# privacy-scaling-explorations/snark-verifier

Hardware: AMD Instinct MI355X
Metric: BN254 G1 MSM points/sec at 2^20 (higher is better)
Workload: dtype i32x9 (254-bit Montgomery Fq as 9 x 29-bit limbs on the integer VALU); 1 GPU; BN254 G1 Pippenger MSM, 2^20 random points/scalars per GPU, inputs resident in HBM, affine result (configs[1]); points_per_gpu=1048576, points_per_kernel_launch=1048576, window_bits=default, msms_in_flight=264

## Files before the change

### snark-verifier_amd/csrc/ctx.hpp

```cpp
#pragma once
#include <hip/hip_runtime.h>
#include <mutex>
#include <stddef.h>
#include <stdint.h>
#include <stdio.h>
#include "../../include/snarkv_amd.h"
#include "curve_consts.h"

#if defined(SNARKV_CURVE_PALLAS)
#define SNARKV_API(name) snarkv_pallas_##name
#define SNARKV_CHUNK_PIPELINE 0
#define SNARKV_API_FLAGS SNARKV_FLAG_VALIDATE
#else
#define SNARKV_API(name) snarkv_##name
#define SNARKV_CHUNK_PIPELINE 1
#define SNARKV_API_FLAGS (SNARKV_FLAG_VALIDATE | SNARKV_FLAG_MONTGOMERY)
#endif

namespace snarkv {

void set_last_error(const char* fmt, ...);

#define SNARKV_HIP(expr)                                                                   \
  do {                                                                                     \
// ... 32 lines not shown
  SLOT_MISC,
  SLOT_SORT_TMP,
  SLOT_SHIFTED,
  SLOT_GLV,
  SLOT_FIX_LISTS,
  SLOT_MISC2,
  SLOT_TERM_CHAIN,
  SLOT_TERM_MAGS,
  SLOT_SPLIT_PARTIALS,
  SLOT_IPA_XI,
  SLOT_IPA_H,
  SLOT_IPA_OUT,
  SLOT_MGPU_GRID,
  SLOT_MGPU_RECV,
  SLOT_IPA_FOLD,
  SLOT_POLY,
  SLOT_NTT,
  SLOT_POLY_PROD,
  SLOT_COUNT
};

}

struct snarkv_ctx {
  int device;
  hipStream_t stream;
  bool own_stream;
  void* buf[snarkv::SLOT_COUNT];
  size_t cap[snarkv::SLOT_COUNT];
  void* hbuf[SNARKV_HOST_BUFFERS];
  size_t hbuf_cap[SNARKV_HOST_BUFFERS];
  uint32_t flags;
  bool mont;
  bool stage_timing;
  float stage_ms[SNARKV_PIP_STAGES];
  hipEvent_t ev[SNARKV_PIP_STAGES + 1];
  bool ev_ready;
  snarkv_ctx* sub[4];
  hipEvent_t sub_ev[5];
  bool sub_ready;
  hipEvent_t sorted_ev;
  bool sorted_ev_ready;
  int last_split_workers;
  bool throughput_mode;
  int throughput_peers;
  bool is_lane;
  snarkv_ctx* jobs[SNARKV_MANY_MAX_JOBS];
  int njobs;
  int last_many_jobs;
  size_t many_sig;
  hipStream_t copy_stream;
  bool copy_ready;
  hipEvent_t many_ev[2];
  hipEvent_t order_ev;
  bool order_ev_ready;
  hipStream_t hi_stream[2];
  bool hi_ready;
  void* ntt_tables;
  uint32_t ntt_key;
};

struct snarkv_dk {
  int device;
// ... 32 lines not shown
  explicit WireFormScope(snarkv_ctx* ctx) : c(ctx), saved(ctx ? ctx->mont : false) {
    if (c) c->mont = false;
  }
  ~WireFormScope() {
    if (c) c->mont = saved;
  }
};
#define SNARKV_WIRE_FORM(ctx) ::snarkv::WireFormScope _wire_form((ctx))

int ctx_reserve(snarkv_ctx* ctx, int slot, size_t bytes, void** out);
int stage_in(snarkv_ctx* ctx, int slot, const void* host, size_t bytes, void** d);
int fetch_out(snarkv_ctx* ctx, const void* d, void* host, size_t bytes);
int check_validate(snarkv_ctx* ctx, const void* d_s, const void* d_p, size_t n, uint32_t flags);
int ctx_lanes(snarkv_ctx* ctx);
int ctx_lanes_fork(snarkv_ctx* ctx);
int ctx_lanes_join(snarkv_ctx* ctx);
inline snarkv_ctx* ctx_lane(snarkv_ctx* ctx, size_t i) { return (i % 4 == 3) ? ctx : ctx->sub[i % 4]; }

int launch_msm_batched(snarkv_ctx* ctx, const void* d_scalars, const void* d_points, const void* d_offsets,
                       size_t n_msm, size_t n_terms, void* d_out);
int launch_g1_decompress(snarkv_ctx* ctx, const void* d_in32, size_t n, void* d_out64, void* d_ok);
int launch_msm_pippenger(snarkv_ctx* ctx, const void* d_scalars, const void* d_points, size_t n, int window_bits,
                         void* d_out, bool partial_out, void* d_buckets_out = nullptr);
enum { PIP_PHASE_SORT = 1, PIP_PHASE_ACC = 2, PIP_PHASE_TAIL = 4, PIP_PHASE_ALL = 7 };
int launch_msm_pippenger_phases(snarkv_ctx* ctx, hipStream_t st, int phases, const void* d_scalars, const void* d_points,
                                size_t n, int window_bits, void* d_out, bool partial_out, void* d_buckets_out,
                                void* d_grid);
int launch_buckets_reduce_many(snarkv_ctx* ctx, hipStream_t st, const void* d_grids, uint32_t c, uint32_t windows,
                               uint32_t jobs, void* d_out, bool partial_out);
int launch_msm_pippenger_many(snarkv_ctx* ctx, size_t count, const void* const* d_scalars, const void* const* d_points,
                              const size_t* n, int window_bits, void* d_out, bool partial_out, hipEvent_t* ready = nullptr);
int launch_msm_pippenger_auto(snarkv_ctx* ctx, const void* d_scalars, const void* d_points, size_t n, int window_bits,
                              void* d_out, bool partial_out);
bool pip_chunk_pipeline(size_t n, int window_bits, bool is_lane, size_t* chunk);
int msm_pippenger_staged(snarkv_ctx* ctx, const uint8_t* scalars32, const uint8_t* points64, size_t n, uint32_t flags,
                         uint8_t out64[64]);
int pip_geometry(size_t n_total, int window_bits, uint32_t* c, uint32_t* windows, uint32_t* buckets_per_window);
int launch_buckets_add(snarkv_ctx* ctx, void* d_dst, const void* d_src, size_t count);
int launch_buckets_reduce(snarkv_ctx* ctx, const void* d_buckets, uint32_t c, uint32_t w0, uint32_t wcount, void* d_partial);
int launch_fold_partials(snarkv_ctx* ctx, const void* d_partials, size_t count, void* d_out64, bool partial_out = false);
int launch_fold_partials_many(snarkv_ctx* ctx, const void* d_partials, size_t count, size_t jobs, void* d_out64s);
constexpr size_t kSharedTableCap = (size_t)256 << 20;
bool ipa_dk_table_fits(const snarkv_ipa_dk* dk);
int ipa_dk_table_prepare(snarkv_ctx* ctx, const snarkv_ipa_dk* dk, bool* have);
int launch_msm_shared(snarkv_ctx* ctx, const snarkv_ipa_dk* dk, const void* d_scalars, size_t n, size_t m, uint32_t slices,
                      void* d_out64s);
int launch_validate(snarkv_ctx* ctx, const void* d_scalars, const void* d_points, size_t n, int* bad_host);
int launch_g2_prepare(snarkv_ctx* ctx, const void* d_g2x2_256, void* d_prep);
int launch_decide(snarkv_ctx* ctx, const void* d_prep, const void* d_accs, size_t m, void* d_ok, void* d_gt);
int launch_validate_g2(snarkv_ctx* ctx, const void* d_g2x2_256, int* bad_host);
// ... 7 lines not shown
```

### snark-verifier_amd/csrc/msm_api.hip

```cpp
#include <stdlib.h>
#include <algorithm>
#include "ctx.hpp"
#include "../../include/snarkv_pallas.h"

namespace snarkv {

bool pip_chunk_pipeline(size_t n, int window_bits, bool is_lane, size_t* chunk) {
  const size_t c = (size_t)1 << 20;
  const char* e = getenv("SNARKV_PIP_SPLIT");
  const int mode = e ? atoi(e) : 1;
  const size_t min_chunks = mode == 2 ? 2 : 3;
  if (chunk) *chunk = c;
  return SNARKV_CHUNK_PIPELINE && mode != 0 && (n + c - 1) / c >= min_chunks && window_bits == 0 && !is_lane;
}

int launch_msm_pippenger_auto(snarkv_ctx* ctx, const void* d_s, const void* d_p, size_t n, int window_bits, void* d_out,
                              bool partial_out) {
  size_t kChunk = 0;
  const bool split = pip_chunk_pipeline(n, window_bits, ctx->is_lane, &kChunk);
  const size_t chunks = (n + kChunk - 1) / kChunk;
  ctx->last_split_workers = 0;
  ctx->last_many_jobs = 0;
  if (!split) return launch_msm_pippenger(ctx, d_s, d_p, n, window_bits, d_out, partial_out);
  SNARKV_TRY(ctx_lanes(ctx));
  const bool tm = ctx->stage_timing;
  if (tm && !ctx->ev_ready) {
// ... 96 lines not shown
    for (int i = 0; i <= SNARKV_PIP_STAGES; ++i) SNARKV_HIP(hipEventCreate(&ctx->ev[i]));
    ctx->ev_ready = true;
  }
  if (sig != ctx->many_sig) {
    SNARKV_HIP(hipDeviceSynchronize());
    ctx->many_sig = sig;
  }
  hipStream_t S[3] = {ctx->stream, ctx->sub[0]->stream, ctx->sub[1]->stream};
  constexpr int nS = 3;
  auto join_and_fork = [&]() -> int {
    for (int k = 0; k < 2; ++k) {
      SNARKV_HIP(hipEventRecord(ctx->many_ev[k], ctx->hi_stream[k]));
      SNARKV_HIP(hipStreamWaitEvent(ctx->stream, ctx->many_ev[k], 0));
    }
    for (int k = 0; k + 1 < nS; ++k) {
      SNARKV_HIP(hipEventRecord(ctx->sub_ev[k], S[k + 1]));
      SNARKV_HIP(hipStreamWaitEvent(ctx->stream, ctx->sub_ev[k], 0));
    }
    SNARKV_HIP(hipEventRecord(ctx->sub_ev[4], ctx->stream));
    for (int k = 0; k < 2; ++k) SNARKV_HIP(hipStreamWaitEvent(ctx->hi_stream[k], ctx->sub_ev[4], 0));
    for (int k = 0; k + 1 < nS; ++k) SNARKV_HIP(hipStreamWaitEvent(S[k + 1], ctx->sub_ev[4], 0));
    return SNARKV_OK;
  };
  void* d_grids = nullptr;
  const size_t grid_bytes = (size_t)w0 * b0 * SNARKV_G1_PARTIAL_BYTES;
  if (uniform) SNARKV_TRY(ctx_reserve(ctx, SLOT_MGPU_GRID, grid_bytes * G, &d_grids));
  if (tm) SNARKV_HIP(hipEventRecord(ctx->ev[0], ctx->stream));
  SNARKV_TRY(join_and_fork());
  for (size_t lo = 0; lo < count; lo += G) {
    const size_t hi = std::min(count, lo + G);
    const bool last = hi == count;
    for (size_t i = lo; i < hi; ++i) {
      snarkv_ctx* job = ctx->jobs[i - lo];
      job->mont = ctx->mont;
      job->stage_timing = tm && last;
      void* grid = uniform ? (uint8_t*)d_grids + grid_bytes * (i - lo) : nullptr;
      hipStream_t sa = ctx->hi_stream[(i - lo) % 2], sb = S[(i - lo) % nS];
      if (ready) SNARKV_HIP(hipStreamWaitEvent(sa, ready[i], 0));
      SNARKV_TRY(launch_msm_pippenger_phases(job, sa, PIP_PHASE_SORT, d_s[i], d_p[i], n[i], window_bits, nullptr, false,
                                             nullptr, grid));
      SNARKV_HIP(hipEventRecord(job->sorted_ev, sa));
      SNARKV_HIP(hipStreamWaitEvent(sb, job->sorted_ev, 0));
      SNARKV_TRY(launch_msm_pippenger_phases(job, sb, PIP_PHASE_ACC, d_s[i], d_p[i], n[i], window_bits, nullptr, false,
                                             nullptr, grid));
      if (!uniform)
        SNARKV_TRY(launch_msm_pippenger_phases(job, sb, PIP_PHASE_TAIL, d_s[i], d_p[i], n[i], window_bits,
                                               (uint8_t*)d_out + ostride * i, partial_out, nullptr, nullptr));
      job->stage_timing = false;
    }
    SNARKV_TRY(join_and_fork());
    if (uniform) {
      SNARKV_TRY(launch_buckets_reduce_many(ctx, ctx->stream, d_grids, c0, w0, (uint32_t)(hi - lo),
                                            (uint8_t*)d_out + ostride * lo, partial_out));
      if (!last) SNARKV_TRY(join_and_fork());
    }
    if (last) ctx->last_many_jobs = (int)(hi - lo);
  }
  if (tm) SNARKV_HIP(hipEventRecord(ctx->ev[SNARKV_PIP_STAGES - 1], ctx->stream));
  return SNARKV_OK;
}

int msm_pippenger_staged(snarkv_ctx* ctx, const uint8_t* scalars32, const uint8_t* points64, size_t n, uint32_t flags,
                         uint8_t out64[64]) {
  if (!ctx || !scalars32 || !points64 || !out64) return SNARKV_ERR_ARG;
  if (n == 0) return SNARKV_ERR_EMPTY;
  SNARKV_HIP(hipSetDevice(ctx->device));
  SNARKV_CALL_FLAGS(ctx, flags & SNARKV_API_FLAGS);
  void *d_s, *d_p, *d_out;
  SNARKV_TRY(stage_in(ctx, SLOT_IN_SCALARS, scalars32, n * 32, &d_s));
  SNARKV_TRY(stage_in(ctx, SLOT_IN_POINTS, points64, n * 64, &d_p));
  SNARKV_TRY(ctx_reserve(ctx, SLOT_OUT, 64, &d_out));
  SNARKV_TRY(check_validate(ctx, d_s, d_p, n, flags));
  SNARKV_TRY(launch_msm_pippenger_auto(ctx, d_s, d_p, n, 0, d_out, false));
// ... 49 lines not shown
```

### snark-verifier_amd/csrc/msm_pippenger.hip

```cpp
#include <stdlib.h>
#include <string.h>
#include <algorithm>
#include <mutex>
#include <atomic>
#include "ctx.hpp"
#include "g1_29.h"
#include "fr29.h"
#ifndef SNARKV_GLV
#define SNARKV_GLV 1
#endif
#if SNARKV_GLV
#include "glv.h"
#endif

namespace snarkv {

#ifndef SNARKV_KRUN
#define SNARKV_KRUN 128
#endif
#ifndef SNARKV_KCHUNK
#define SNARKV_KCHUNK 8
#endif
#ifndef SNARKV_TILE_THREADS
#define SNARKV_TILE_THREADS 256
// ... 116 lines not shown
    k[4 * j + 1] = q.y;
    k[4 * j + 2] = q.z;
    k[4 * j + 3] = q.w;
  }
#if SNARKV_GLV
  uint32_t sgn = k[3] >> 31;
  k[3] &= 0x7FFFFFFFu;
  return sgn;
#else
  return 0u;
#endif
}

__device__ __forceinline__ uint32_t xcd_tile(uint32_t b, uint32_t nblk) {
#if SNARKV_XCD_TILES
  return (nblk & 7u) == 0 ? (b & 7u) * (nblk >> 3) + (b >> 3) : b;
#else
  return b;
#endif
}

__global__ void __launch_bounds__(SNARKV_PREP_THREADS)
    k_prepare(const uint32_t* __restrict__ scalars, const uint32_t* __restrict__ points,
              G1Packed* __restrict__ pts, uint4* __restrict__ glv, PipParams p, uint32_t* __restrict__ M) {
  SNARKV_RAISE_PRIO();
  extern __shared__ uint32_t lds[];
  for (uint32_t k = threadIdx.x; k < p.nkeys; k += blockDim.x) lds[k] = 0u;
  __syncthreads();
  const uint32_t tile = xcd_tile(blockIdx.x, p.nblk);
  uint32_t lo = tile * p.tile;
  uint32_t hi = lo + p.tile < p.n ? lo + p.tile : p.n;
  for (uint32_t i = lo + threadIdx.x; i < hi; i += blockDim.x) {
    const uint4* s = reinterpret_cast<const uint4*>(points + (size_t)i * 16);
    uint32_t w[16];
#pragma unroll
    for (int j = 0; j < 4; ++j) {
      uint4 v = s[j];
      w[4 * j] = v.x;
      w[4 * j + 1] = v.y;
      w[4 * j + 2] = v.z;
      w[4 * j + 3] = v.w;
    }
    G1Affine29 a = g1a29_from_words(w, p.mont != 0);
    bool ident = g1a29_is_identity(a);
    pts[kHalves * (size_t)i] = g1a29_pack(a);
    const uint4* ks = reinterpret_cast<const uint4*>(scalars + (size_t)i * 8);
    uint4 k0 = ks[0], k1 = ks[1];
// ... 13 lines not shown
    pts[2 * (size_t)i + 1] = g1a29_pack(a);
    glv_decompose(k, o);
#else
#pragma unroll
    for (int j = 0; j < 8; ++j) o[j] = k[j];
#endif
    if (ident) {
#pragma unroll
      for (int j = 0; j < 8; ++j) o[j] = 0;
    }
    glv[2 * (size_t)i] = make_uint4(o[0], o[1], o[2], o[3]);
    glv[2 * (size_t)i + 1] = make_uint4(o[4], o[5], o[6], o[7]);
#pragma unroll
    for (int h = 0; h < kHalves; ++h) {
      uint32_t d[kDigitWords];
      uint32_t sgn = load_digit_words(o + h * kDigitWords, d);
      for_each_digit(d, sgn, p, [&](uint32_t key, uint32_t, uint32_t) { atomicAdd(&lds[key], 1u); });
    }
  }
  __syncthreads();
  for (uint32_t k = threadIdx.x; k < p.nkeys; k += blockDim.x) M[(size_t)k * p.mstride + tile] = lds[k];
  if (blockIdx.x == 0 && p.mstride > p.nblk)
    for (uint32_t k = threadIdx.x; k < p.nkeys; k += blockDim.x) M[(size_t)k * p.mstride + p.nblk] = 0u;
}

constexpr uint32_t kStageScalars = SNARKV_TILE_BASE;
constexpr uint32_t kStageItems = kStageScalars / SNARKV_TILE_THREADS;
static_assert(kStageScalars % SNARKV_TILE_THREADS == 0, "a staged tile gives every lane the same number of scalars");
__global__ void __launch_bounds__(SNARKV_TILE_THREADS) SNARKV_SCATTER_ATTR
    k_sort_scatter_staged(const uint4* __restrict__ glv, PipParams p, const uint32_t* __restrict__ M,
                          uint2* __restrict__ tmp) {
  SNARKV_RAISE_PRIO();
  extern __shared__ uint32_t lds[];
  uint32_t* gbase = lds;
  uint32_t* cnt = lds + p.SB;
  uint32_t* off = lds + 2 * p.SB;
  uint32_t* wsum = lds + 3 * p.SB;
  uint2* stage = reinterpret_cast<uint2*>(lds + 3 * p.SB + 16 + (p.SB & 1u));
  const uint32_t tid = threadIdx.x, lane = tid & 63u, wave = tid >> 6;
  const uint32_t tile = xcd_tile(blockIdx.x, p.nblk);
  const uint32_t lo = tile * kStageScalars;
  const uint32_t hi = lo + kStageScalars < p.n ? lo + kStageScalars : p.n;
  const uint32_t per = (p.SB + SNARKV_TILE_THREADS - 1) / SNARKV_TILE_THREADS;
  for (int w = 0; w < p.W; ++w) {
    for (uint32_t k = tid; k < p.SB; k += blockDim.x) {
      gbase[k] = M[((size_t)w * p.SB + k) * p.mstride + tile];
// ... 182 lines not shown
    for (int j = 0; j < kPer; ++j) {
      uint32_t e = threadIdx.x + j * T;
      if (e < cnt_items) stage[atomicAdd(&hist[mine[j].x & low_mask], 1u)] = mine[j];
    }
    __syncthreads();
    for (uint32_t e = threadIdx.x; e < cnt_items; e += T) entries[begin + e] = stage[e];
  } else {
    for (uint32_t e = begin + threadIdx.x; e < end; e += T) {
      uint2 it = tmp[e];
      entries[begin + atomicAdd(&hist[it.x & low_mask], 1u)] = it;
    }
  }
}

constexpr uint32_t kSchedBuckets = 2048;
constexpr uint32_t kMaxPiece = 256;
constexpr uint32_t kBigPieces = 24;
constexpr uint32_t kFixGrid = 1024;
constexpr uint32_t kPieceWhole = 0x80000000u;
__host__ __device__ constexpr uint32_t sched_rows(uint32_t L) { return L + 3; }

__global__ void __launch_bounds__(256)
    k_piece_hist(const uint32_t* __restrict__ counts, PipParams p, uint32_t nsb, uint32_t* __restrict__ H,
                 uint32_t* __restrict__ misc) {
  SNARKV_RAISE_PRIO();
  __shared__ uint32_t hist[sched_rows(kMaxPiece)];
  const uint32_t L = p.krun, rows = sched_rows(L);
  for (uint32_t k = threadIdx.x; k < rows; k += blockDim.x) hist[k] = 0u;
  if (blockIdx.x == 0 && threadIdx.x == 0) misc[4] = 0u;
  __syncthreads();
  const uint32_t lo = blockIdx.x * kSchedBuckets, hi = lo + kSchedBuckets < p.nb ? lo + kSchedBuckets : p.nb;
  for (uint32_t b = lo + threadIdx.x; b < hi; b += blockDim.x) {
    const uint32_t c = counts[b];
    if (c <= L) {
      atomicAdd(&hist[L - c], 1u);
      continue;
    }
    const uint32_t nfull = c / L, r = c - nfull * L;
    atomicAdd(&hist[0], nfull);
    if (r) atomicAdd(&hist[L - r], 1u);
    atomicAdd(&hist[nfull + (r ? 1u : 0u) > kBigPieces ? L + 2 : L + 1], 1u);
  }
  __syncthreads();
  for (uint32_t k = threadIdx.x; k < rows; k += blockDim.x) H[(size_t)k * nsb + blockIdx.x] = hist[k];
}

__global__ void __launch_bounds__(256)
    k_piece_emit(const uint32_t* __restrict__ counts, const uint32_t* __restrict__ offsets, PipParams p, uint32_t nsb,
                 const uint32_t* __restrict__ H, uint32_t split_slots, uint4* __restrict__ pieces,
                 uint32_t* __restrict__ small_list, uint32_t* __restrict__ big_list) {
  SNARKV_RAISE_PRIO();
  __shared__ uint32_t cur[sched_rows(kMaxPiece)];
  const uint32_t L = p.krun, rows = sched_rows(L);
  for (uint32_t k = threadIdx.x; k < rows; k += blockDim.x) cur[k] = H[(size_t)k * nsb + blockIdx.x];
  const uint32_t small0 = H[(size_t)(L + 1) * nsb], big0 = H[(size_t)(L + 2) * nsb];
  __syncthreads();
  const uint32_t lo = blockIdx.x * kSchedBuckets, hi = lo + kSchedBuckets < p.nb ? lo + kSchedBuckets : p.nb;
  for (uint32_t b = lo + threadIdx.x; b < hi; b += blockDim.x) {
    const uint32_t c = counts[b], o = offsets[b];
    if (c <= L) {
      pieces[atomicAdd(&cur[L - c], 1u)] = make_uint4(o, c | kPieceWhole, b, 0u);
      continue;
    }
    const uint32_t nfull = c / L, r = c - nfull * L, slot = o / L;
    const uint32_t at = atomicAdd(&cur[0], nfull);
    for (uint32_t j = 0; j < nfull; ++j) pieces[at + j] = make_uint4(o + j * L, L, b, slot + j);
    if (r) pieces[atomicAdd(&cur[L - r], 1u)] = make_uint4(o + nfull * L, r, b, split_slots + slot);
    if (nfull + (r ? 1u : 0u) > kBigPieces) big_list[atomicAdd(&cur[L + 2], 1u) - big0] = b;
    else small_list[atomicAdd(&cur[L + 1], 1u) - small0] = b;
  }
}

constexpr uint32_t kEntryIdx = 0x7FFFFFFFu;

__device__ __forceinline__ G1Affine29 entry_point(const G1Packed& k, uint32_t y) {
  G1Affine29 p = g1a29_unpack(k);
  if (y >> 31) p.y = fq29_neg(p.y);
  return p;
}
// ... 56 lines not shown
    const uint32_t i = atomicAdd(deg_count, 1u);
    if (i < p.nb) deg_list[i] = b;
  } else {
    buckets[b] = acc;
  }
}

__device__ __noinline__ void bucket_from_entries_careful(const uint2* __restrict__ entries, const G1Packed* __restrict__ pts,
                                                         uint32_t o, uint32_t cnt, uint32_t first, uint32_t stride,
                                                         bool sanitize, G1Xyzz29* out) {
  G1Xyzz29 acc = xyzz29_identity();
  for (uint32_t e = o + first; e < o + cnt; e += stride) {
    uint2 ent = entries[e];
    G1Affine29 p = entry_point(pts[ent.y & kEntryIdx], ent.y);
    xyzz29_madd_careful(acc, p);
  }
  *out = sanitize ? xyzz29_sanitize(acc) : acc;
}

__device__ __forceinline__ uint32_t piece_slot(uint32_t o, uint32_t j, uint32_t nfull, uint32_t L, uint32_t split_slots) {
  return j < nfull ? o / L + j : split_slots + o / L;
}

__global__ void __launch_bounds__(256)
    k_fixup(const uint32_t* __restrict__ counts, const uint32_t* __restrict__ offsets, const uint2* __restrict__ entries,
            const G1Packed* __restrict__ pts, const G1Xyzz29* __restrict__ parts, uint32_t split_slots,
            G1Xyzz29* __restrict__ buckets, const uint32_t* __restrict__ H, uint32_t nsb, const uint32_t* __restrict__ misc,
            const uint32_t* __restrict__ small_list, const uint32_t* __restrict__ big_list,
            const uint32_t* __restrict__ deg_list, PipParams p) {
  SNARKV_RAISE_PRIO();
  __shared__ G1Xyzz29 sh[256];
  __shared__ int any_bad;
  const uint32_t L = p.krun;
  const uint32_t small0 = H[(size_t)(L + 1) * nsb], big0 = H[(size_t)(L + 2) * nsb];
  const uint32_t nsmall = big0 - small0, nbig = misc[6] - big0;
  const uint32_t ndeg = misc[4] < p.nb ? misc[4] : p.nb;
  for (uint32_t bi = blockIdx.x; bi < nbig; bi += gridDim.x) {
    const uint32_t b = big_list[bi];
    const uint32_t o = offsets[b], cnt = counts[b], nfull = cnt / L, np = nfull + (cnt % L ? 1u : 0u);
    if (threadIdx.x == 0) any_bad = 0;
    __syncthreads();
    G1Xyzz29 acc = xyzz29_identity();
    bool bad = false;
    for (uint32_t j = threadIdx.x; j < np; j += blockDim.x) {
      const G1Xyzz29 part = parts[piece_slot(o, j, nfull, L, split_slots)];
      bad = bad || xyzz29_is_degenerate(part);
      xyzz29_add_careful(acc, part);
    }
    if (bad) atomicOr(&any_bad, 1);
    __syncthreads();
    if (any_bad) bucket_from_entries_careful(entries, pts, o, cnt, threadIdx.x, blockDim.x, false, &sh[threadIdx.x]);
    else sh[threadIdx.x] = acc;
    __syncthreads();
    for (uint32_t st = 128; st >= 1; st >>= 1) {
      if (threadIdx.x < st) {
        G1Xyzz29 a = sh[threadIdx.x];
        xyzz29_add_careful(a, sh[threadIdx.x + st]);
        sh[threadIdx.x] = a;
      }
      __syncthreads();
    }
    if (threadIdx.x == 0) buckets[b] = xyzz29_sanitize(sh[0]);
    __syncthreads();
  }
  for (uint32_t i = blockIdx.x * blockDim.x + threadIdx.x; i < nsmall + ndeg; i += gridDim.x * blockDim.x) {
    const bool split = i < nsmall;
    const uint32_t b = split ? small_list[i] : deg_list[i - nsmall];
    const uint32_t o = offsets[b], cnt = counts[b];
    bool bad = !split;
    G1Xyzz29 acc = xyzz29_identity();
    if (split) {
      const uint32_t nfull = cnt / L, np = nfull + (cnt % L ? 1u : 0u);
      for (uint32_t j = 0; j < np; ++j) {
        const G1Xyzz29 part = parts[piece_slot(o, j, nfull, L, split_slots)];
        bad = bad || xyzz29_is_identity(part);
        xyzz29_add_skipid_fast(acc, part, bad);
      }
      bad = bad || xyzz29_is_degenerate(acc);
    }
    if (bad) bucket_from_entries_careful(entries, pts, o, cnt, 0, 1, true, &buckets[b]);
    else buckets[b] = acc;
  }
}

__device__ __forceinline__ G1Xyzz29 xyzz29_sel(bool c, const G1Xyzz29& a, const G1Xyzz29& b) {
  G1Xyzz29 r;
#pragma unroll
  for (int i = 0; i < 9; ++i) {
    r.x.v[i] = c ? a.x.v[i] : b.x.v[i];
    r.y.v[i] = c ? a.y.v[i] : b.y.v[i];
    r.zz.v[i] = c ? a.zz.v[i] : b.zz.v[i];
    r.zzz.v[i] = c ? a.zzz.v[i] : b.zzz.v[i];
  }
  return r;
}

template <bool CAREFUL>
__device__ __forceinline__ bool chunk_sums(const G1Xyzz29* __restrict__ bw, uint32_t base, uint32_t top,
                                           G1Xyzz29& run, G1Xyzz29& acc) {
  run = xyzz29_identity();
  acc = xyzz29_identity();
  bool bad = false;
#pragma unroll 1
  for (uint32_t op = 0; op < 2 * (top - base); ++op) {
    bool second = op & 1u;
// ... 209 lines not shown
  while (high < p.c - 1 && ((kHalves * n) >> (high + 1)) >= kSortTarget && ((uint64_t)p.W << (high + 1)) <= kMaxKeys) ++high;
  p.low_bits = (p.c - 1) - high;
  p.SB = p.B >> p.low_bits;
  p.nkeys = (uint32_t)p.W * p.SB;
  p.tile = SNARKV_TILE_BASE;
  static_assert(kStageItems * kHalves <= 32, "a staged lane keeps one sign bit per entry in a 32-bit word");
  const size_t lds_staged = ((size_t)3 * p.SB + 16 + (p.SB & 1u)) * 4 + (size_t)kStageScalars * kHalves * 8;
  p.nblk = (uint32_t)((n + p.tile - 1) / p.tile);
  p.mstride = p.nblk | 1u;
  uint64_t max_entries = (uint64_t)kHalves * (uint64_t)n * (uint64_t)p.W;
  if (n == 0 || max_entries >= 0xFFFFFFFFull || n >= 0x40000000ull) {
    set_last_error("pippenger: n=%zu out of range", n);
    return SNARKV_ERR_LENGTH;
  }
  if ((size_t)p.nkeys * 4 > 65536 || lds_staged > 96 * 1024) {
    set_last_error("pippenger: key table too large (nkeys=%u)", p.nkeys);
    return SNARKV_ERR_LENGTH;
  }
  p.krun = ctx->throughput_mode ? (uint32_t)kRunThroughput : latency_run_length(max_entries);
  const uint32_t max_pieces = (uint32_t)std::min<uint64_t>((uint64_t)p.nb + max_entries / p.krun, 0xFFFFFFFFull - 63);
  const uint32_t split_slots = (uint32_t)(max_entries / p.krun) + 1;
  const uint32_t nsb = (p.nb + kSchedBuckets - 1) / kSchedBuckets;
  const uint32_t hcount = sched_rows(p.krun) * nsb;
  const uint32_t hscan_blocks = (hcount + 1023) / 1024;
  uint32_t mcount = p.nkeys * p.mstride;
  uint32_t scan_blocks = (mcount + 1023) / 1024;
  uint32_t chunks_per_window = (p.B + kChunk - 1) / kChunk;
  uint32_t blocks_per_window = (chunks_per_window + 63) / 64;

  void *d_pts, *d_glv, *d_counts, *d_offsets, *d_M, *d_blocksum, *d_entries, *d_tmp, *d_pieces, *d_hist, *d_parts,
      *d_buckets, *d_wave, *d_shift, *d_misc, *d_lists;
  SNARKV_TRY(ctx_reserve(ctx, SLOT_POINTS_MONT, kHalves * n * sizeof(G1Packed), &d_pts));
  SNARKV_TRY(ctx_reserve(ctx, SLOT_GLV, n * 32, &d_glv));
  SNARKV_TRY(ctx_reserve(ctx, SLOT_COUNTS, (size_t)p.nb * 4, &d_counts));
  SNARKV_TRY(ctx_reserve(ctx, SLOT_OFFSETS, (size_t)p.nb * 4, &d_offsets));
  SNARKV_TRY(ctx_reserve(ctx, SLOT_CURSOR, (size_t)mcount * 4, &d_M));
  SNARKV_TRY(ctx_reserve(ctx, SLOT_BLOCKSUMS, (size_t)std::max(scan_blocks, hscan_blocks) * 4 + 64, &d_blocksum));
  SNARKV_TRY(ctx_reserve(ctx, SLOT_ENTRIES, max_entries * 8, &d_entries));
  SNARKV_TRY(ctx_reserve(ctx, SLOT_SORT_TMP, max_entries * 8, &d_tmp));
  SNARKV_TRY(ctx_reserve(ctx, SLOT_PIECES, (size_t)max_pieces * sizeof(uint4), &d_pieces));
  SNARKV_TRY(ctx_reserve(ctx, SLOT_PIECE_HIST, (size_t)hcount * 4, &d_hist));
  SNARKV_TRY(ctx_reserve(ctx, SLOT_SPLIT_PARTS, (size_t)split_slots * 2 * sizeof(G1Xyzz29), &d_parts));
  if (d_grid) d_buckets = d_grid;
  else SNARKV_TRY(ctx_reserve(ctx, SLOT_BUCKETS, (size_t)p.nb * sizeof(G1Xyzz29), &d_buckets));
  SNARKV_TRY(ctx_reserve(ctx, SLOT_CHUNK_PARTIALS, 2 * (size_t)blocks_per_window * p.W * sizeof(G1Xyzz29), &d_wave));
  SNARKV_TRY(ctx_reserve(ctx, SLOT_SHIFTED, (size_t)p.W * sizeof(G1Xyzz29), &d_shift));
  SNARKV_TRY(ctx_reserve(ctx, SLOT_MISC, 64, &d_misc));
  SNARKV_TRY(ctx_reserve(ctx, SLOT_FIX_LISTS, (size_t)p.nb * 3 * 4, &d_lists));
  uint32_t* d_total = (uint32_t*)d_misc;
  uint32_t* d_small = (uint32_t*)d_lists, *d_bigl = d_small + p.nb, *d_deg = d_bigl + p.nb;
  const uint32_t* d_npieces = (const uint32_t*)d_hist + (size_t)(p.krun + 1) * nsb;

  const bool tm = ctx->stage_timing && phases == PIP_PHASE_ALL;
  const bool tm_acc = ctx->stage_timing && phases == PIP_PHASE_ACC;
  int evi = 0;
#define STAGE_MARK()                                         \
  do {                                                       \
    if (tm) SNARKV_HIP(hipEventRecord(ctx->ev[evi++], st));  \
  } while (0)
  if ((tm || tm_acc) && !ctx->ev_ready) {
    for (int i = 0; i <= SNARKV_PIP_STAGES; ++i) SNARKV_HIP(hipEventCreate(&ctx->ev[i]));
    ctx->ev_ready = true;
  }
  STAGE_MARK();
  if (phases & PIP_PHASE_SORT) {
    hipLaunchKernelGGL(k_prepare, dim3(p.nblk), dim3(SNARKV_PREP_THREADS), (size_t)p.nkeys * 4, st, (const uint32_t*)d_scalars,
                       (const uint32_t*)d_points, (G1Packed*)d_pts, (uint4*)d_glv, p, (uint32_t*)d_M);
    STAGE_MARK();
    hipLaunchKernelGGL(k_scan_local, dim3(scan_blocks), dim3(256), 0, st, (uint32_t*)d_M, (uint32_t*)d_blocksum, mcount);
    hipLaunchKernelGGL(k_scan_blocksums, dim3(1), dim3(1024), 0, st, (uint32_t*)d_blocksum, scan_blocks, d_total);
    hipLaunchKernelGGL(k_scan_add, dim3(scan_blocks), dim3(256), 0, st, (uint32_t*)d_M, (const uint32_t*)d_blocksum,
                       mcount);
    STAGE_MARK();
    static std::atomic<uint64_t> attr_set{0};
    const uint64_t bit = 1ull << (ctx->device & 63);
    if (!(attr_set.load(std::memory_order_relaxed) & bit)) {
      SNARKV_HIP(hipFuncSetAttribute(reinterpret_cast<const void*>(k_sort_scatter_staged),
                                     hipFuncAttributeMaxDynamicSharedMemorySize, 96 * 1024));
      attr_set.fetch_or(bit, std::memory_order_relaxed);
    }
    hipLaunchKernelGGL(k_sort_scatter_staged, dim3(p.nblk), dim3(SNARKV_TILE_THREADS), lds_staged, st, (const uint4*)d_glv,
                       p, (const uint32_t*)d_M, (uint2*)d_tmp);
    const uint32_t nbins_l2 = 1u << p.low_bits;
    const size_t lds2 = ((size_t)nbins_l2 + SNARKV_L2_THREADS + 1) * 4 + (size_t)kSortCap * 8;
    hipLaunchKernelGGL(k_sort_level2, dim3(p.nkeys), dim3(SNARKV_L2_THREADS), lds2, st, (const uint2*)d_tmp, (const uint32_t*)d_M,
                       d_total, p, (uint2*)d_entries, (uint32_t*)d_counts, (uint32_t*)d_offsets);
    hipLaunchKernelGGL(k_piece_hist, dim3(nsb), dim3(256), 0, st, (const uint32_t*)d_counts, p, nsb, (uint32_t*)d_hist,
                       d_total);
    hipLaunchKernelGGL(k_scan_local, dim3(hscan_blocks), dim3(256), 0, st, (uint32_t*)d_hist, (uint32_t*)d_blocksum, hcount);
    hipLaunchKernelGGL(k_scan_blocksums, dim3(1), dim3(1024), 0, st, (uint32_t*)d_blocksum, hscan_blocks, d_total + 6);
    hipLaunchKernelGGL(k_scan_add, dim3(hscan_blocks), dim3(256), 0, st, (uint32_t*)d_hist, (const uint32_t*)d_blocksum,
                       hcount);
    hipLaunchKernelGGL(k_piece_emit, dim3(nsb), dim3(256), 0, st, (const uint32_t*)d_counts, (const uint32_t*)d_offsets, p,
                       nsb, (const uint32_t*)d_hist, split_slots, (uint4*)d_pieces, d_small, d_bigl);
  }
  STAGE_MARK();
  if (tm_acc) SNARKV_HIP(hipEventRecord(ctx->ev[3], st));
  if (phases & PIP_PHASE_ACC)
    hipLaunchKernelGGL(k_accumulate, dim3((max_pieces + 63) / 64), dim3(64), 0, st, (const uint4*)d_pieces, d_npieces,
                       (const uint32_t*)d_total, (const uint2*)d_entries, (const G1Packed*)d_pts, (G1Xyzz29*)d_buckets,
                       (G1Xyzz29*)d_parts, 2 * split_slots, d_total + 4, d_deg, p);
  STAGE_MARK();
  if (tm_acc) SNARKV_HIP(hipEventRecord(ctx->ev[4], st));
  if (phases & PIP_PHASE_ACC) {
    const uint64_t split_bound = std::min<uint64_t>(p.nb, max_entries / (p.krun + 1) + 1);
    const uint32_t fix_grid = (uint32_t)std::min<uint64_t>((split_bound + 255) / 256, kFixGrid);
    hipLaunchKernelGGL(k_fixup, dim3(fix_grid), dim3(256), 0, st, (const uint32_t*)d_counts, (const uint32_t*)d_offsets,
                       (const uint2*)d_entries, (const G1Packed*)d_pts, (const G1Xyzz29*)d_parts, split_slots,
                       (G1Xyzz29*)d_buckets, (const uint32_t*)d_hist, nsb, (const uint32_t*)d_total,
                       (const uint32_t*)d_small, (const uint32_t*)d_bigl, (const uint32_t*)d_deg, p);
    if (tm_acc) SNARKV_HIP(hipEventRecord(ctx->ev[5], st));
  }
  STAGE_MARK();
  if (d_buckets_out) {
    if (phases & PIP_PHASE_ACC)
      SNARKV_HIP(hipMemcpyAsync(d_buckets_out, d_buckets, (size_t)p.nb * sizeof(G1Xyzz29), hipMemcpyDeviceToDevice, st));
    SNARKV_HIP(hipGetLastError());
    return SNARKV_OK;
  }
  if (phases & PIP_PHASE_TAIL)
    hipLaunchKernelGGL(k_bucket_reduce, dim3(blocks_per_window * p.W), dim3(64), 0, st, (const G1Xyzz29*)d_buckets,
                       (G1Xyzz29*)d_wave, p, chunks_per_window, blocks_per_window);
  STAGE_MARK();
  if (phases & PIP_PHASE_TAIL)
    hipLaunchKernelGGL(k_shift_windows, dim3(p.W), dim3(64), 0, st, (const G1Xyzz29*)d_wave, (G1Xyzz29*)d_shift, p,
                       blocks_per_window);
  STAGE_MARK();
  if (phases & PIP_PHASE_TAIL)
    hipLaunchKernelGGL(k_final, dim3(1), dim3(64), 0, st, (const G1Xyzz29*)d_shift, (uint32_t)p.W, (uint32_t*)d_out,
                       partial_out ? 1 : 0, p.mont);
  STAGE_MARK();
#undef STAGE_MARK
  SNARKV_HIP(hipGetLastError());
  return SNARKV_OK;
}
// ... 29 lines not shown
  PipParams p;
  memset(&p, 0, sizeof p);
  p.c = (int)c;
  p.W = (int)wcount;
  p.B = 1u << (c - 1);
  p.nb = wcount * p.B;
  p.w0 = w0;
  p.chunk_log2 = (uint32_t)kLog2Chunk;
  uint32_t chunks_per_window = (p.B + kChunk - 1) / kChunk;
  uint32_t blocks_per_window = (chunks_per_window + 63) / 64;
  void *d_wave, *d_shift;
  SNARKV_TRY(ctx_reserve(ctx, SLOT_CHUNK_PARTIALS, 2 * (size_t)blocks_per_window * wcount * sizeof(G1Xyzz29), &d_wave));
  SNARKV_TRY(ctx_reserve(ctx, SLOT_SHIFTED, (size_t)wcount * sizeof(G1Xyzz29), &d_shift));
  hipStream_t st = ctx->stream;
  hipLaunchKernelGGL(k_bucket_reduce, dim3(blocks_per_window * wcount), dim3(64), 0, st, (const G1Xyzz29*)d_buckets,
                     (G1Xyzz29*)d_wave, p, chunks_per_window, blocks_per_window);
  hipLaunchKernelGGL(k_shift_windows, dim3(wcount), dim3(64), 0, st, (const G1Xyzz29*)d_wave, (G1Xyzz29*)d_shift, p,
                     blocks_per_window);
  hipLaunchKernelGGL(k_final, dim3(1), dim3(64), 0, st, (const G1Xyzz29*)d_shift, wcount, (uint32_t*)d_partial, 1, 0u);
  SNARKV_HIP(hipGetLastError());
  return SNARKV_OK;
}

struct TailGeom {
  PipParams p;
  uint32_t chunks_per_window, blocks_per_window;
  void *d_wave, *d_shift;
};
static int tail_geometry(snarkv_ctx* ctx, uint32_t c, uint32_t windows, uint32_t jobs, TailGeom* g) {
  PipParams& p = g->p;
  memset(&p, 0, sizeof p);
  p.c = (int)c;
  p.W = (int)(windows * jobs);
  p.B = 1u << (c - 1);
  p.nb = windows * jobs * p.B;
  p.w0 = 0;
  p.wper = windows;
  const uint32_t wtotal = windows * jobs;
  uint32_t cl2 = (uint32_t)kLog2Chunk;
  {
    static int slots = 0;
    if (!slots) {
      hipDeviceProp_t prop;
      slots = hipGetDeviceProperties(&prop, ctx->device) == hipSuccess && prop.multiProcessorCount > 0 ? 8 * prop.multiProcessorCount : 2048;
    }
    uint64_t best = ~0ull;
// ... 33 lines not shown
```

Measured before the change: 784.5 million points/s.

## Batch bucket fixup across MSM jobs and replace piece-histogram scan with atomic row totals

Moves the per-job k_fixup launch out of each lane's accumulate phase into batched k_fixup_many_lanes/k_fixup_many_big kernels that handle up to 16 jobs per launch on the main stream before the uniform bucket reduce. Separately, it replaces the three-kernel global scan of the piece histogram with per-row atomic totals in k_piece_hist plus an in-block prefix over row totals inside k_piece_emit, which now writes the list starts into misc. This is meant to cut launch count and small-kernel overhead when many MSMs are in flight, at the cost of non-deterministic piece ordering from the atomics and serializing fixup on the main stream after the join.

```diff
diff --git a/snark-verifier_amd/csrc/ctx.hpp b/snark-verifier_amd/csrc/ctx.hpp
--- a/snark-verifier_amd/csrc/ctx.hpp
+++ b/snark-verifier_amd/csrc/ctx.hpp
@@ -78,6 +78,20 @@
 
 }
 
+struct snarkv_fix_job {
+  const void* counts;
+  const void* offsets;
+  const void* entries;
+  const void* pts;
+  const void* parts;
+  const void* misc;
+  const void* lists;
+  void* buckets;
+  uint32_t split_slots, nb, krun;
+  uint32_t split_bound;
+};
+constexpr int kFixJobsPerLaunch = 16;
+
 struct snarkv_ctx {
   int device;
   hipStream_t stream;
@@ -95,6 +109,7 @@
   snarkv_ctx* sub[4];
   hipEvent_t sub_ev[5];
   bool sub_ready;
+  snarkv_fix_job fix;
   hipEvent_t sorted_ev;
   bool sorted_ev_ready;
   int last_split_workers;
@@ -173,10 +188,11 @@
 int launch_g1_decompress(snarkv_ctx* ctx, const void* d_in32, size_t n, void* d_out64, void* d_ok);
 int launch_msm_pippenger(snarkv_ctx* ctx, const void* d_scalars, const void* d_points, size_t n, int window_bits,
                          void* d_out, bool partial_out, void* d_buckets_out = nullptr);
-enum { PIP_PHASE_SORT = 1, PIP_PHASE_ACC = 2, PIP_PHASE_TAIL = 4, PIP_PHASE_ALL = 7 };
+enum { PIP_PHASE_SORT = 1, PIP_PHASE_ACC = 2, PIP_PHASE_TAIL = 4, PIP_PHASE_FIX = 8, PIP_PHASE_ALL = 15 };
 int launch_msm_pippenger_phases(snarkv_ctx* ctx, hipStream_t st, int phases, const void* d_scalars, const void* d_points,
                                 size_t n, int window_bits, void* d_out, bool partial_out, void* d_buckets_out,
                                 void* d_grid);
+int launch_fixup_many(hipStream_t st, snarkv_ctx* const* jobs, size_t count);
 int launch_buckets_reduce_many(snarkv_ctx* ctx, hipStream_t st, const void* d_grids, uint32_t c, uint32_t windows,
                                uint32_t jobs, void* d_out, bool partial_out);
 int launch_msm_pippenger_many(snarkv_ctx* ctx, size_t count, const void* const* d_scalars, const void* const* d_points,
diff --git a/snark-verifier_amd/csrc/msm_api.hip b/snark-verifier_amd/csrc/msm_api.hip
--- a/snark-verifier_amd/csrc/msm_api.hip
+++ b/snark-verifier_amd/csrc/msm_api.hip
@@ -2,6 +2,10 @@
 #include <algorithm>
 #include "ctx.hpp"
 #include "../../include/snarkv_pallas.h"
+
+#ifndef SNARKV_FIXUP_IN_TAIL
+#define SNARKV_FIXUP_IN_TAIL 1
+#endif
 
 namespace snarkv {
 
@@ -144,6 +148,7 @@
     for (int k = 0; k + 1 < nS; ++k) SNARKV_HIP(hipStreamWaitEvent(S[k + 1], ctx->sub_ev[4], 0));
     return SNARKV_OK;
   };
+  const bool fix_in_tail = uniform && SNARKV_FIXUP_IN_TAIL;
   void* d_grids = nullptr;
   const size_t grid_bytes = (size_t)w0 * b0 * SNARKV_G1_PARTIAL_BYTES;
   if (uniform) SNARKV_TRY(ctx_reserve(ctx, SLOT_MGPU_GRID, grid_bytes * G, &d_grids));
@@ -163,14 +168,15 @@
                                              nullptr, grid));
       SNARKV_HIP(hipEventRecord(job->sorted_ev, sa));
       SNARKV_HIP(hipStreamWaitEvent(sb, job->sorted_ev, 0));
-      SNARKV_TRY(launch_msm_pippenger_phases(job, sb, PIP_PHASE_ACC, d_s[i], d_p[i], n[i], window_bits, nullptr, false,
-                                             nullptr, grid));
+      SNARKV_TRY(launch_msm_pippenger_phases(job, sb, fix_in_tail ? PIP_PHASE_ACC : PIP_PHASE_ACC | PIP_PHASE_FIX, d_s[i],
+                                             d_p[i], n[i], window_bits, nullptr, false, nullptr, grid));
       if (!uniform)
         SNARKV_TRY(launch_msm_pippenger_phases(job, sb, PIP_PHASE_TAIL, d_s[i], d_p[i], n[i], window_bits,
                                                (uint8_t*)d_out + ostride * i, partial_out, nullptr, nullptr));
       job->stage_timing = false;
     }
     SNARKV_TRY(join_and_fork());
+    if (fix_in_tail) SNARKV_TRY(launch_fixup_many(ctx->stream, ctx->jobs, hi - lo));
     if (uniform) {
       SNARKV_TRY(launch_buckets_reduce_many(ctx, ctx->stream, d_grids, c0, w0, (uint32_t)(hi - lo),
                                             (uint8_t*)d_out + ostride * lo, partial_out));
diff --git a/snark-verifier_amd/csrc/msm_pippenger.hip b/snark-verifier_amd/csrc/msm_pippenger.hip
--- a/snark-verifier_amd/csrc/msm_pippenger.hip
+++ b/snark-verifier_amd/csrc/msm_pippenger.hip
@@ -162,7 +162,8 @@
 
 __global__ void __launch_bounds__(SNARKV_PREP_THREADS)
     k_prepare(const uint32_t* __restrict__ scalars, const uint32_t* __restrict__ points,
-              G1Packed* __restrict__ pts, uint4* __restrict__ glv, PipParams p, uint32_t* __restrict__ M) {
+              G1Packed* __restrict__ pts, uint4* __restrict__ glv, PipParams p, uint32_t* __restrict__ M,
+              uint32_t* __restrict__ rowtot) {
   SNARKV_RAISE_PRIO();
   extern __shared__ uint32_t lds[];
   for (uint32_t k = threadIdx.x; k < p.nkeys; k += blockDim.x) lds[k] = 0u;
@@ -222,6 +223,8 @@
   for (uint32_t k = threadIdx.x; k < p.nkeys; k += blockDim.x) M[(size_t)k * p.mstride + tile] = lds[k];
   if (blockIdx.x == 0 && p.mstride > p.nblk)
     for (uint32_t k = threadIdx.x; k < p.nkeys; k += blockDim.x) M[(size_t)k * p.mstride + p.nblk] = 0u;
+  if (blockIdx.x == 0)
+    for (uint32_t k = threadIdx.x; k < p.krun + 3; k += blockDim.x) rowtot[k] = 0u;
 }
 
 constexpr uint32_t kStageScalars = SNARKV_TILE_BASE;
@@ -450,7 +453,7 @@
 
 __global__ void __launch_bounds__(256)
     k_piece_hist(const uint32_t* __restrict__ counts, PipParams p, uint32_t nsb, uint32_t* __restrict__ H,
-                 uint32_t* __restrict__ misc) {
+                 uint32_t* __restrict__ rowtot, uint32_t* __restrict__ misc) {
   SNARKV_RAISE_PRIO();
   __shared__ uint32_t hist[sched_rows(kMaxPiece)];
   const uint32_t L = p.krun, rows = sched_rows(L);
@@ -470,19 +473,57 @@
     atomicAdd(&hist[nfull + (r ? 1u : 0u) > kBigPieces ? L + 2 : L + 1], 1u);
   }
   __syncthreads();
-  for (uint32_t k = threadIdx.x; k < rows; k += blockDim.x) H[(size_t)k * nsb + blockIdx.x] = hist[k];
+  for (uint32_t k = threadIdx.x; k < rows; k += blockDim.x)
+    H[(size_t)k * nsb + blockIdx.x] = hist[k] ? atomicAdd(&rowtot[k], hist[k]) : 0u;
 }
 
 __global__ void __launch_bounds__(256)
     k_piece_emit(const uint32_t* __restrict__ counts, const uint32_t* __restrict__ offsets, PipParams p, uint32_t nsb,
-                 const uint32_t* __restrict__ H, uint32_t split_slots, uint4* __restrict__ pieces,
-                 uint32_t* __restrict__ small_list, uint32_t* __restrict__ big_list) {
+                 const uint32_t* __restrict__ H, const uint32_t* __restrict__ rowtot, uint32_t split_slots,
+                 uint4* __restrict__ pieces, uint32_t* __restrict__ small_list, uint32_t* __restrict__ big_list,
+                 uint32_t* __restrict__ misc) {
   SNARKV_RAISE_PRIO();
   __shared__ uint32_t cur[sched_rows(kMaxPiece)];
+  __shared__ uint32_t wsum[4];
+  __shared__ uint32_t list0[3];
   const uint32_t L = p.krun, rows = sched_rows(L);
-  for (uint32_t k = threadIdx.x; k < rows; k += blockDim.x) cur[k] = H[(size_t)k * nsb + blockIdx.x];
-  const uint32_t small0 = H[(size_t)(L + 1) * nsb], big0 = H[(size_t)(L + 2) * nsb];
-  __syncthreads();
+  const uint32_t tid = threadIdx.x, lane = tid & 63u, wave = tid >> 6;
+  const uint32_t per = (rows + 255) / 256;
+  uint32_t tot[2] = {0u, 0u}, mine = 0;
+#pragma unroll
+  for (uint32_t j = 0; j < 2; ++j) {
+    const uint32_t k = tid * per + j;
+    if (j < per && k < rows) tot[j] = rowtot[k];
+    mine += tot[j];
+  }
+  uint32_t incl = mine;
+#pragma unroll
+  for (int d = 1; d < 64; d <<= 1) {
+    const uint32_t up = __shfl_up(incl, d, 64);
+    if ((int)lane >= d) incl += up;
+  }
+  if (lane == 63) wsum[wave] = incl;
+  __syncthreads();
+  uint32_t run = incl - mine;
+  for (uint32_t q = 0; q < wave; ++q) run += wsum[q];
+#pragma unroll
+  for (uint32_t j = 0; j < 2; ++j) {
+    const uint32_t k = tid * per + j;
+    if (j < per && k < rows) {
+      if (k == L + 1) list0[0] = run;
+      if (k == L + 2) list0[1] = run;
+      cur[k] = run + H[(size_t)k * nsb + blockIdx.x];
+      run += tot[j];
+    }
+  }
+  if (tid == 255) list0[2] = run;
+  __syncthreads();
+  const uint32_t small0 = list0[0], big0 = list0[1];
+  if (blockIdx.x == 0 && tid == 0) {
+    misc[5] = small0;
+    misc[7] = big0;
+    misc[6] = list0[2];
+  }
   const uint32_t lo = blockIdx.x * kSchedBuckets, hi = lo + kSchedBuckets < p.nb ? lo + kSchedBuckets : p.nb;
   for (uint32_t b = lo + threadIdx.x; b < hi; b += blockDim.x) {
     const uint32_t c = counts[b], o = offsets[b];
@@ -585,34 +626,52 @@
   return j < nfull ? o / L + j : split_slots + o / L;
 }
 
-__global__ void __launch_bounds__(256)
-    k_fixup(const uint32_t* __restrict__ counts, const uint32_t* __restrict__ offsets, const uint2* __restrict__ entries,
-            const G1Packed* __restrict__ pts, const G1Xyzz29* __restrict__ parts, uint32_t split_slots,
-            G1Xyzz29* __restrict__ buckets, const uint32_t* __restrict__ H, uint32_t nsb, const uint32_t* __restrict__ misc,
-            const uint32_t* __restrict__ small_list, const uint32_t* __restrict__ big_list,
-            const uint32_t* __restrict__ deg_list, PipParams p) {
-  SNARKV_RAISE_PRIO();
-  __shared__ G1Xyzz29 sh[256];
-  __shared__ int any_bad;
-  const uint32_t L = p.krun;
-  const uint32_t small0 = H[(size_t)(L + 1) * nsb], big0 = H[(size_t)(L + 2) * nsb];
-  const uint32_t nsmall = big0 - small0, nbig = misc[6] - big0;
-  const uint32_t ndeg = misc[4] < p.nb ? misc[4] : p.nb;
-  for (uint32_t bi = blockIdx.x; bi < nbig; bi += gridDim.x) {
-    const uint32_t b = big_list[bi];
-    const uint32_t o = offsets[b], cnt = counts[b], nfull = cnt / L, np = nfull + (cnt % L ? 1u : 0u);
-    if (threadIdx.x == 0) any_bad = 0;
+struct FixLists {
+  const uint32_t *counts, *offsets, *small_list, *big_list, *deg_list;
+  const uint2* entries;
+  const G1Packed* pts;
+  const G1Xyzz29* parts;
+  G1Xyzz29* buckets;
+  uint32_t L, split_slots, nsmall, nbig, ndeg;
+};
+__device__ __forceinline__ FixLists fix_lists(const snarkv_fix_job& j) {
+  FixLists f;
+  const uint32_t* misc = (const uint32_t*)j.misc;
+  const uint32_t small0 = misc[5], big0 = misc[7];
+  f.counts = (const uint32_t*)j.counts;
+  f.offsets = (const uint32_t*)j.offsets;
+  f.small_list = (const uint32_t*)j.lists;
+  f.big_list = f.small_list + j.nb;
+  f.deg_list = f.big_list + j.nb;
+  f.entries = (const uint2*)j.entries;
+  f.pts = (const G1Packed*)j.pts;
+  f.parts = (const G1Xyzz29*)j.parts;
+  f.buckets = (G1Xyzz29*)j.buckets;
+  f.L = j.krun;
+  f.split_slots = j.split_slots;
+  f.nsmall = min(big0 - small0, j.nb);
+  f.nbig = min(misc[6] - big0, j.nb);
+  f.ndeg = min(misc[4], j.nb);
+  return f;
+}
+
+__device__ __forceinline__ void fixup_big(const FixLists& f, G1Xyzz29* sh, int* any_bad, uint32_t wg, uint32_t nwg) {
+  const uint32_t L = f.L;
+  for (uint32_t bi = wg; bi < f.nbig; bi += nwg) {
+    const uint32_t b = f.big_list[bi];
+    const uint32_t o = f.offsets[b], cnt = f.counts[b], nfull = cnt / L, np = nfull + (cnt % L ? 1u : 0u);
+    if (threadIdx.x == 0) *any_bad = 0;
     __syncthreads();
     G1Xyzz29 acc = xyzz29_identity();
     bool bad = false;
-    for (uint32_t j = threadIdx.x; j < np; j += blockDim.x) {
-      const G1Xyzz29 part = parts[piece_slot(o, j, nfull, L, split_slots)];
+    for (uint32_t j = threadIdx.x; j < np; j += 256) {
+      const G1Xyzz29 part = f.parts[piece_slot(o, j, nfull, L, f.split_slots)];
       bad = bad || xyzz29_is_degenerate(part);
       xyzz29_add_careful(acc, part);
     }
-    if (bad) atomicOr(&any_bad, 1);
-    __syncthreads();
-    if (any_bad) bucket_from_entries_careful(entries, pts, o, cnt, threadIdx.x, blockDim.x, false, &sh[threadIdx.x]);
+    if (bad) atomicOr(any_bad, 1);
+    __syncthreads();
+    if (*any_bad) bucket_from_entries_careful(f.entries, f.pts, o, cnt, threadIdx.x, 256, false, &sh[threadIdx.x]);
     else sh[threadIdx.x] = acc;
     __syncthreads();
     for (uint32_t st = 128; st >= 1; st >>= 1) {
@@ -623,27 +682,56 @@
       }
       __syncthreads();
     }
-    if (threadIdx.x == 0) buckets[b] = xyzz29_sanitize(sh[0]);
-    __syncthreads();
-  }
-  for (uint32_t i = blockIdx.x * blockDim.x + threadIdx.x; i < nsmall + ndeg; i += gridDim.x * blockDim.x) {
-    const bool split = i < nsmall;
-    const uint32_t b = split ? small_list[i] : deg_list[i - nsmall];
-    const uint32_t o = offsets[b], cnt = counts[b];
+    if (threadIdx.x == 0) f.buckets[b] = xyzz29_sanitize(sh[0]);
+    __syncthreads();
+  }
+}
+
+__device__ __forceinline__ void fixup_lanes(const FixLists& f, uint32_t first, uint32_t nlanes) {
+  const uint32_t L = f.L;
+  for (uint32_t i = first; i < f.nsmall + f.ndeg; i += nlanes) {
+    const bool split = i < f.nsmall;
+    const uint32_t b = split ? f.small_list[i] : f.deg_list[i - f.nsmall];
+    const uint32_t o = f.offsets[b], cnt = f.counts[b];
     bool bad = !split;
     G1Xyzz29 acc = xyzz29_identity();
     if (split) {
       const uint32_t nfull = cnt / L, np = nfull + (cnt % L ? 1u : 0u);
       for (uint32_t j = 0; j < np; ++j) {
-        const G1Xyzz29 part = parts[piece_slot(o, j, nfull, L, split_slots)];
+        const G1Xyzz29 part = f.parts[piece_slot(o, j, nfull, L, f.split_slots)];
         bad = bad || xyzz29_is_identity(part);
         xyzz29_add_skipid_fast(acc, part, bad);
       }
       bad = bad || xyzz29_is_degenerate(acc);
     }
-    if (bad) bucket_from_entries_careful(entries, pts, o, cnt, 0, 1, true, &buckets[b]);
-    else buckets[b] = acc;
-  }
+    if (bad) bucket_from_entries_careful(f.entries, f.pts, o, cnt, 0, 1, true, &f.buckets[b]);
+    else f.buckets[b] = acc;
+  }
+}
+
+__global__ void __launch_bounds__(256) k_fixup(snarkv_fix_job job) {
+  SNARKV_RAISE_PRIO();
+  __shared__ G1Xyzz29 sh[256];
+  __shared__ int any_bad;
+  const FixLists f = fix_lists(job);
+  fixup_big(f, sh, &any_bad, blockIdx.x, gridDim.x);
+  fixup_lanes(f, blockIdx.x * 256 + threadIdx.x, gridDim.x * 256);
+}
+
+struct FixBatch {
+  snarkv_fix_job job[kFixJobsPerLaunch];
+};
+__global__ void __launch_bounds__(64) k_fixup_many_lanes(FixBatch batch) {
+  SNARKV_RAISE_PRIO();
+  const FixLists f = fix_lists(batch.job[blockIdx.y]);
+  fixup_lanes(f, blockIdx.x * 64 + threadIdx.x, gridDim.x * 64);
+}
+__global__ void __launch_bounds__(256) k_fixup_many_big(FixBatch batch) {
+  SNARKV_RAISE_PRIO();
+  __shared__ G1Xyzz29 sh[256];
+  __shared__ int any_bad;
+  const FixLists f = fix_lists(batch.job[blockIdx.y]);
+  fixup_big(f, sh, &any_bad, blockIdx.x, gridDim.x);
 }
 
 __device__ __forceinline__ G1Xyzz29 xyzz29_sel(bool c, const G1Xyzz29& a, const G1Xyzz29& b) {
@@ -899,7 +987,6 @@
   const uint32_t split_slots = (uint32_t)(max_entries / p.krun) + 1;
   const uint32_t nsb = (p.nb + kSchedBuckets - 1) / kSchedBuckets;
   const uint32_t hcount = sched_rows(p.krun) * nsb;
-  const uint32_t hscan_blocks = (hcount + 1023) / 1024;
   uint32_t mcount = p.nkeys * p.mstride;
   uint32_t scan_blocks = (mcount + 1023) / 1024;
   uint32_t chunks_per_window = (p.B + kChunk - 1) / kChunk;
@@ -912,11 +999,11 @@
   SNARKV_TRY(ctx_reserve(ctx, SLOT_COUNTS, (size_t)p.nb * 4, &d_counts));
   SNARKV_TRY(ctx_reserve(ctx, SLOT_OFFSETS, (size_t)p.nb * 4, &d_offsets));
   SNARKV_TRY(ctx_reserve(ctx, SLOT_CURSOR, (size_t)mcount * 4, &d_M));
-  SNARKV_TRY(ctx_reserve(ctx, SLOT_BLOCKSUMS, (size_t)std::max(scan_blocks, hscan_blocks) * 4 + 64, &d_blocksum));
+  SNARKV_TRY(ctx_reserve(ctx, SLOT_BLOCKSUMS, (size_t)scan_blocks * 4 + 64, &d_blocksum));
   SNARKV_TRY(ctx_reserve(ctx, SLOT_ENTRIES, max_entries * 8, &d_entries));
   SNARKV_TRY(ctx_reserve(ctx, SLOT_SORT_TMP, max_entries * 8, &d_tmp));
   SNARKV_TRY(ctx_reserve(ctx, SLOT_PIECES, (size_t)max_pieces * sizeof(uint4), &d_pieces));
-  SNARKV_TRY(ctx_reserve(ctx, SLOT_PIECE_HIST, (size_t)hcount * 4, &d_hist));
+  SNARKV_TRY(ctx_reserve(ctx, SLOT_PIECE_HIST, ((size_t)hcount + sched_rows(p.krun)) * 4, &d_hist));
   SNARKV_TRY(ctx_reserve(ctx, SLOT_SPLIT_PARTS, (size_t)split_slots * 2 * sizeof(G1Xyzz29), &d_parts));
   if (d_grid) d_buckets = d_grid;
   else SNARKV_TRY(ctx_reserve(ctx, SLOT_BUCKETS, (size_t)p.nb * sizeof(G1Xyzz29), &d_buckets));
@@ -926,10 +1013,11 @@
   SNARKV_TRY(ctx_reserve(ctx, SLOT_FIX_LISTS, (size_t)p.nb * 3 * 4, &d_lists));
   uint32_t* d_total = (uint32_t*)d_misc;
   uint32_t* d_small = (uint32_t*)d_lists, *d_bigl = d_small + p.nb, *d_deg = d_bigl + p.nb;
-  const uint32_t* d_npieces = (const uint32_t*)d_hist + (size_t)(p.krun + 1) * nsb;
+  const uint32_t* d_npieces = d_total + 5;
+  uint32_t* d_rowtot = (uint32_t*)d_hist + hcount;
 
   const bool tm = ctx->stage_timing && phases == PIP_PHASE_ALL;
-  const bool tm_acc = ctx->stage_timing && phases == PIP_PHASE_ACC;
+  const bool tm_acc = ctx->stage_timing && (phases & ~PIP_PHASE_FIX) == PIP_PHASE_ACC;
   int evi = 0;
 #define STAGE_MARK()                                         \
   do {                                                       \
@@ -942,7 +1030,7 @@
   STAGE_MARK();
   if (phases & PIP_PHASE_SORT) {
     hipLaunchKernelGGL(k_prepare, dim3(p.nblk), dim3(SNARKV_PREP_THREADS), (size_t)p.nkeys * 4, st, (const uint32_t*)d_scalars,
-                       (const uint32_t*)d_points, (G1Packed*)d_pts, (uint4*)d_glv, p, (uint32_t*)d_M);
+                       (const uint32_t*)d_points, (G1Packed*)d_pts, (uint4*)d_glv, p, (uint32_t*)d_M, d_rowtot);
     STAGE_MARK();
     hipLaunchKernelGGL(k_scan_local, dim3(scan_blocks), dim3(256), 0, st, (uint32_t*)d_M, (uint32_t*)d_blocksum, mcount);
     hipLaunchKernelGGL(k_scan_blocksums, dim3(1), dim3(1024), 0, st, (uint32_t*)d_blocksum, scan_blocks, d_total);
@@ -963,13 +1051,10 @@
     hipLaunchKernelGGL(k_sort_level2, dim3(p.nkeys), dim3(SNARKV_L2_THREADS), lds2, st, (const uint2*)d_tmp, (const uint32_t*)d_M,
                        d_total, p, (uint2*)d_entries, (uint32_t*)d_counts, (uint32_t*)d_offsets);
     hipLaunchKernelGGL(k_piece_hist, dim3(nsb), dim3(256), 0, st, (const uint32_t*)d_counts, p, nsb, (uint32_t*)d_hist,
-                       d_total);
-    hipLaunchKernelGGL(k_scan_local, dim3(hscan_blocks), dim3(256), 0, st, (uint32_t*)d_hist, (uint32_t*)d_blocksum, hcount);
-    hipLaunchKernelGGL(k_scan_blocksums, dim3(1), dim3(1024), 0, st, (uint32_t*)d_blocksum, hscan_blocks, d_total + 6);
-    hipLaunchKernelGGL(k_scan_add, dim3(hscan_blocks), dim3(256), 0, st, (uint32_t*)d_hist, (const uint32_t*)d_blocksum,
-                       hcount);
+                       d_rowtot, d_total);
     hipLaunchKernelGGL(k_piece_emit, dim3(nsb), dim3(256), 0, st, (const uint32_t*)d_counts, (const uint32_t*)d_offsets, p,
-                       nsb, (const uint32_t*)d_hist, split_slots, (uint4*)d_pieces, d_small, d_bigl);
+                       nsb, (const uint32_t*)d_hist, (const uint32_t*)d_rowtot, split_slots, (uint4*)d_pieces, d_small,
+                       d_bigl, d_total);
   }
   STAGE_MARK();
   if (tm_acc) SNARKV_HIP(hipEventRecord(ctx->ev[3], st));
@@ -980,14 +1065,17 @@
   STAGE_MARK();
   if (tm_acc) SNARKV_HIP(hipEventRecord(ctx->ev[4], st));
   if (phases & PIP_PHASE_ACC) {
-    const uint64_t split_bound = std::min<uint64_t>(p.nb, max_entries / (p.krun + 1) + 1);
-    const uint32_t fix_grid = (uint32_t)std::min<uint64_t>((split_bound + 255) / 256, kFixGrid);
-    hipLaunchKernelGGL(k_fixup, dim3(fix_grid), dim3(256), 0, st, (const uint32_t*)d_counts, (const uint32_t*)d_offsets,
-                       (const uint2*)d_entries, (const G1Packed*)d_pts, (const G1Xyzz29*)d_parts, split_slots,
-                       (G1Xyzz29*)d_buckets, (const uint32_t*)d_hist, nsb, (const uint32_t*)d_total,
-                       (const uint32_t*)d_small, (const uint32_t*)d_bigl, (const uint32_t*)d_deg, p);
-    if (tm_acc) SNARKV_HIP(hipEventRecord(ctx->ev[5], st));
-  }
+    snarkv_fix_job& f = ctx->fix;
+    f.counts = d_counts, f.offsets = d_offsets, f.entries = d_entries, f.pts = d_pts, f.parts = d_parts, f.misc = d_total;
+    f.lists = d_lists, f.buckets = d_buckets;
+    f.split_slots = split_slots, f.nb = p.nb, f.krun = p.krun;
+    f.split_bound = (uint32_t)std::min<uint64_t>(p.nb, max_entries / (p.krun + 1) + 1);
+  }
+  if (phases & PIP_PHASE_FIX) {
+    const uint32_t fix_grid = std::min<uint32_t>((ctx->fix.split_bound + 255) / 256, kFixGrid);
+    hipLaunchKernelGGL(k_fixup, dim3(fix_grid), dim3(256), 0, st, ctx->fix);
+  }
+  if (tm_acc) SNARKV_HIP(hipEventRecord(ctx->ev[5], st));
   STAGE_MARK();
   if (d_buckets_out) {
     if (phases & PIP_PHASE_ACC)
@@ -1063,6 +1151,27 @@
   return SNARKV_OK;
 }
 
+constexpr uint32_t kFixLaneGrid = 256, kFixBigGrid = 64;
+int launch_fixup_many(hipStream_t st, snarkv_ctx* const* jobs, size_t count) {
+  for (size_t lo = 0; lo < count; lo += kFixJobsPerLaunch) {
+    const uint32_t m = (uint32_t)std::min<size_t>(kFixJobsPerLaunch, count - lo);
+    FixBatch b;
+    uint32_t split_bound = 1, big_bound = 1;
+    for (uint32_t k = 0; k < (uint32_t)kFixJobsPerLaunch; ++k) {
+      b.job[k] = jobs[lo + (k < m ? k : 0)]->fix;
+      if (k < m) {
+        split_bound = std::max(split_bound, b.job[k].split_bound);
+        big_bound = std::max(big_bound, (uint32_t)((uint64_t)b.job[k].split_bound * (b.job[k].krun + 1) /
+                                                   ((uint64_t)(kBigPieces - 1) * b.job[k].krun + 1) + 1));
+      }
+    }
+    hipLaunchKernelGGL(k_fixup_many_lanes, dim3(std::min((split_bound + 63) / 64, kFixLaneGrid), m), dim3(64), 0, st, b);
+    hipLaunchKernelGGL(k_fixup_many_big, dim3(std::min(big_bound, kFixBigGrid), m), dim3(256), 0, st, b);
+  }
+  SNARKV_HIP(hipGetLastError());
+  return SNARKV_OK;
+}
+
 struct TailGeom {
   PipParams p;
   uint32_t chunks_per_window, blocks_per_window;
```

Measured after the change: 776.3 million points/s. 1.0% lower.
